# liangyuwang/Tiny-DeepSpeed

Hardware: AMD Instinct MI355X
Metric: tokens/sec (whole node) GPT-2 ZeRO-2 (higher is better)
Workload: dtype bf16; 1 GPU; model=gpt2-medium, global_batch=32, seq_len=1024, parallelism=zero2-dp1

## Files before the change

### csrc/kernels/attention.hip

```cpp
#include "common.h"
#include "launchers.h"
#include "mfma.h"

#include <type_traits>

namespace tdsa {

constexpr int KVB = 64;
constexpr int D = 64;
constexpr float LOG2E = 1.4426950408889634f;
constexpr float LN2 = 0.6931471805599453f;

DEV_INLINE float fast_exp2(float x) { return __builtin_amdgcn_exp2f(x); }
DEV_INLINE float fast_rcp(float x) { return __builtin_amdgcn_rcpf(x); }

DEV_INLINE void xcd_remap(int gx, long long gy, int& tile, long long& bh) {
  if (gy % 8 == 0) {
    const long long id = bh * gx + tile;
    tile = (int)((id % (8 * gx)) / 8);
    bh = (id / (8 * gx)) * 8 + (id % 8);
  }
}

struct GStride {
  long long b;
  long long h;
  int t;
};

struct BlockCtx {
  int tile;
  long long bh;
  int tid, lane, w;
  int x32, h32;

  DEV_INLINE BlockCtx() {
    tile = blockIdx.x;
    bh = blockIdx.y;
    xcd_remap(gridDim.x, gridDim.y, tile, bh);
    tid = threadIdx.x;
    lane = tid & (WAVE - 1);
    w = tid / WAVE;
    x32 = lane & 31;
    h32 = lane >> 5;
  }

  DEV_INLINE long long base(const GStride& s, int H) const {
    return (bh / H) * s.b + (bh % H) * s.h;
  }
};

struct FragOff {
  int row[2];
  int xk;
  int h16;

  DEV_INLINE FragOff(const BlockCtx& c)
      : row{c.x32 * 128, (32 + c.x32) * 128}, xk((c.x32 & 7) << 4),
        h16(16 * c.h32) {}

  DEV_INLINE int operator()(int t2, int s) const {
    return row[t2] + ((s * 32 + h16) ^ xk);
  }
};

template <int NT>
struct TilePipe {
  Stage<NT> a, b;
  short8v pend_a[Stage<NT>::REPS], pend_b[Stage<NT>::REPS];

  DEV_INLINE TilePipe(const bf16* ga, int st_a, const bf16* gb, int st_b,
                      int tid)
      : a(ga, tid, st_a), b(gb, tid, st_b) {}

  DEV_INLINE void prime() {
    a.fetch(pend_a);
    b.fetch(pend_b);
  }

  DEV_INLINE void next(char* lds_a, char* lds_b, bool more) {
    __syncthreads();
    a.put(lds_a, pend_a);
    b.put(lds_b, pend_b);
    if (more) {
      a.advance();
      b.advance();
      a.fetch(pend_a);
      b.fetch(pend_b);
    }
  }
};

struct Dropout {
  unsigned long long seed;
  unsigned keep_thr;
  float inv_keep;

  DEV_INLINE bool keep(unsigned long long idx) const {
    unsigned h = (unsigned)(idx ^ (idx >> 32));
    h += (unsigned)seed;
    h ^= (unsigned)(seed >> 32);
    h ^= h >> 16;
    h *= 0x85EBCA6Bu;
    h ^= h >> 13;
    h *= 0xC2B2AE35u;
    h ^= h >> 16;
    return h < keep_thr;
  }
};

struct PackedC {
  unsigned wA[2][4];
  unsigned wB[2][4];
};

DEV_INLINE bfrag frag_from_packed(const PackedC& p, int s) {
  const unsigned uA = p.wA[s >> 1][2 * (s & 1)];
  const unsigned vA = p.wA[s >> 1][2 * (s & 1) + 1];
  const unsigned uB = p.wB[s >> 1][2 * (s & 1)];
  const unsigned vB = p.wB[s >> 1][2 * (s & 1) + 1];
  auto rA = __builtin_amdgcn_permlane32_swap(uA, vA, false, false);
  auto rB = __builtin_amdgcn_permlane32_swap(uB, vB, false, false);
  union { bfrag f; unsigned w[4]; } r;
  r.w[0] = rA[0];
  r.w[1] = rB[0];
  r.w[2] = rA[1];
  r.w[3] = rB[1];
  return r.f;
}

DEV_INLINE bfrag load_frag_scaled(const bf16* p, int row, int col, int st,
                                  float s) {
  short8v v = load8(p + (long long)row * st + col);
  union { bfrag f; short w[8]; } r;
#pragma unroll
  for (int e = 0; e < 8; ++e) r.w[e] = bf_pack(bf_elem(v, e) * s);
  return r.f;
}

DEV_INLINE bfrag load_frag(const bf16* p, int row, int col, int st) {
  union { bfrag f; short8v v; } r;
  r.v = load8(p + (long long)row * st + col);
  return r.f;
}

template <typename F>
DEV_INLINE void store_ctiles(bf16* p, int st, const BlockCtx& c,
                             const f32x16 (&acc)[2], F mul) {
#pragma unroll
  for (int dt = 0; dt < 2; ++dt)
#pragma unroll
    for (int r = 0; r < 16; ++r)
      p[crow(r, c.h32) * st + dt * 32 + c.x32] = f2bf(acc[dt][r] * mul(r));
}

constexpr int fwd_min_blocks(int nw, bool drop) {
  return nw == 8 ? (drop ? 3 : 4) : 2;
}

template <int NW, bool DROP = false>
__launch_bounds__(NW * WAVE, fwd_min_blocks(NW, DROP))
__global__ void attn_fwd_kernel(const bf16* __restrict__ q,
                                const bf16* __restrict__ k,
                                const bf16* __restrict__ v,
                                bf16* __restrict__ o, float* __restrict__ lse,
                                int T, int H, float scale, GStride sq,
                                GStride so, Dropout drop) {
  constexpr int BM = NW * 32;
  constexpr int NT = NW * WAVE;
  __shared__ __attribute__((aligned(16))) char smem[2 * KVB * D * 2];
  char* lds_k = smem;
  char* lds_v = smem + KVB * D * 2;

  const BlockCtx c;
  const long long boff = c.base(sq, H);
  const bf16* qp = q + boff + (long long)(c.tile * BM) * sq.t;

  TilePipe<NT> pipe(k + boff, sq.t, v + boff, sq.t, c.tid);
  const FragOff kf(c);
  int trb[2][2];
  tr_bases(c.lane, trb);
  const float qscale = scale * LOG2E;
  bfrag q_frag[4];
#pragma unroll
  for (int s = 0; s < 4; ++s)
    q_frag[s] = load_frag_scaled(qp, c.w * 32 + c.x32, s * 16 + 8 * c.h32,
                                 sq.t, qscale);

  const f32x16 kzero = {};
  f32x16 o_acc[2] = {};
  float m_run = -INFINITY;
  float l_run = 0.f;

  const int row_lo = c.tile * BM + c.w * 32;
  const int row_me = row_lo + c.x32;
  const unsigned long long drop_base =
      DROP ? ((unsigned long long)c.bh * T + row_me) * T : 0;
  const int n_kv = (c.tile + 1) * BM / KVB;
  pipe.prime();
  for (int j = 0; j < n_kv; ++j) {
    pipe.next(lds_k, lds_v, j + 1 < n_kv);
    __syncthreads();

    const int key0 = j * KVB;
    if (key0 > row_lo + 31) continue;

    f32x16 st[2];
    __builtin_amdgcn_s_setprio(1);
#pragma unroll
    for (int t2 = 0; t2 < 2; ++t2) {
      f32x16 acc = MFMA32(lds_read16(lds_k, kf(t2, 0)), q_frag[0], kzero);
#pragma unroll
      for (int s = 1; s < 4; ++s)
        acc = MFMA32(lds_read16(lds_k, kf(t2, s)), q_frag[s], acc);
      st[t2] = acc;
    }
    __builtin_amdgcn_s_setprio(0);

    const bool diag = key0 + KVB - 1 > row_lo;
    float mt = -INFINITY;
    if (diag) {
#pragma unroll
      for (int t2 = 0; t2 < 2; ++t2)
#pragma unroll
        for (int r = 0; r < 16; ++r) {
          const int key = key0 + t2 * 32 + crow(r, c.h32);
          float s = (key <= row_me) ? st[t2][r] : -INFINITY;
          st[t2][r] = s;
          mt = fmaxf(mt, s);
        }
    } else {
#pragma unroll
      for (int t2 = 0; t2 < 2; ++t2)
#pragma unroll
        for (int r = 0; r < 16; ++r) mt = fmaxf(mt, st[t2][r]);
    }
    mt = fmaxf(mt, __shfl_xor(mt, 32, WAVE));
    const float m_new = fmaxf(m_run, mt);
    const float alpha = fast_exp2(m_run - m_new);
    float psum = 0.f;
    PackedC P;
#pragma unroll
    for (int t2 = 0; t2 < 2; ++t2)
#pragma unroll
      for (int r1 = 0; r1 < 4; ++r1) {
        float p[4];
#pragma unroll
        for (int e = 0; e < 4; ++e) {
          float pe = fast_exp2(st[t2][4 * r1 + e] - m_new);
          psum += pe;
          if (DROP) {
            const int key = key0 + t2 * 32 + crow(4 * r1 + e, c.h32);
            pe = drop.keep(drop_base + key) ? pe * drop.inv_keep : 0.f;
          }
          p[e] = pe;
        }
        P.wA[t2][r1] = pack2(p[0], p[1]);
        P.wB[t2][r1] = pack2(p[2], p[3]);
      }
    psum += __shfl_xor(psum, 32, WAVE);
    l_run = l_run * alpha + psum;
    m_run = m_new;

    if (__any(alpha != 1.0f)) {
      float a_row[16];
#pragma unroll
      for (int r = 0; r < 16; ++r)
        a_row[r] = __shfl(alpha, crow(r, c.h32), WAVE);
#pragma unroll
      for (int dt = 0; dt < 2; ++dt)
#pragma unroll
        for (int r = 0; r < 16; ++r) o_acc[dt][r] *= a_row[r];
    }

    __builtin_amdgcn_s_setprio(1);
#pragma unroll
    for (int s = 0; s < 4; ++s) {
      const bfrag pa = frag_from_packed(P, s);
#pragma unroll
      for (int dt = 0; dt < 2; ++dt)
        o_acc[dt] = MFMA32(pa, tr_bfrag(lds_v, trb[dt][0] + s * 2048,
                                        trb[dt][1] + s * 2048),
                           o_acc[dt]);
    }
    __builtin_amdgcn_s_setprio(0);
  }

  float linv_row[16];
#pragma unroll
  for (int r = 0; r < 16; ++r)
    linv_row[r] = fast_rcp(__shfl(l_run, crow(r, c.h32), WAVE));
  store_ctiles(o + c.base(so, H) + (long long)row_lo * so.t, so.t, c, o_acc,
               [&](int r) { return linv_row[r]; });
  if (c.lane < 32) {
    lse[c.bh * T + row_me] = (m_run + log2f(l_run)) * LN2;
  }
}

template <int NW, bool DROP = false>
__launch_bounds__(NW * WAVE)
__global__ void attn_bwd_dkv_kernel(const bf16* __restrict__ q,
                                    const bf16* __restrict__ k,
                                    const bf16* __restrict__ v,
                                    const bf16* __restrict__ dout,
                                    const float* __restrict__ lse,
                                    const float* __restrict__ delta,
                                    bf16* __restrict__ dk, bf16* __restrict__ dv,
                                    int T, int H, float scale, GStride sq,
                                    GStride so, GStride sd, Dropout drop) {
  constexpr int BK = NW * 32;
  constexpr int NT = NW * WAVE;
  __shared__ __attribute__((aligned(16))) char smem[2 * KVB * D * 2 + 2 * KVB * 4];
  char* lds_q = smem;
  char* lds_do = smem + KVB * D * 2;
  float* lds_lse = reinterpret_cast<float*>(smem + 2 * KVB * D * 2);
  float* lds_dlt = lds_lse + KVB;

  const BlockCtx c;
  const long long boff = c.base(sq, H);
  const int i0 = c.tile * BK / KVB;

  TilePipe<NT> pipe(q + boff + (long long)(i0 * KVB) * sq.t, sq.t,
                    dout + c.base(so, H) + (long long)(i0 * KVB) * so.t, so.t,
                    c.tid);
  const FragOff af(c);
  int trb[2][2];
  tr_bases(c.lane, trb);
  const float kscale = scale * LOG2E;
  const int key_lo = c.tile * BK + c.w * 32;
  const int key_me = key_lo + c.x32;
  const unsigned long long drop_bhTT =
      DROP ? (unsigned long long)c.bh * T * T : 0;
  bfrag k_frag[4], v_frag[4];
#pragma unroll
  for (int s = 0; s < 4; ++s) {
    k_frag[s] = load_frag_scaled(k + boff, key_me, s * 16 + 8 * c.h32, sq.t,
                                 kscale);
    v_frag[s] = load_frag(v + boff, key_me, s * 16 + 8 * c.h32, sq.t);
  }

  const f32x16 kzero = {};
  f32x16 dk_acc[2] = {};
  f32x16 dv_acc[2] = {};

  pipe.prime();
  for (int i = i0; i < T / KVB; ++i) {
    pipe.next(lds_q, lds_do, i + 1 < T / KVB);
    if (c.tid < KVB) {
      lds_lse[c.tid] = lse[c.bh * T + i * KVB + c.tid] * LOG2E;
      lds_dlt[c.tid] = delta[c.bh * T + i * KVB + c.tid];
    }
    __syncthreads();

    const int q0 = i * KVB;
    if (q0 + KVB - 1 < key_lo) continue;

    const bool diag = q0 < key_lo + 32;
    PackedC P, dS;
#pragma unroll
    for (int t2 = 0; t2 < 2; ++t2) {
      __builtin_amdgcn_s_setprio(1);
      f32x16 s_acc = MFMA32(lds_read16(lds_q, af(t2, 0)), k_frag[0], kzero);
      f32x16 dp_acc = MFMA32(lds_read16(lds_do, af(t2, 0)), v_frag[0], kzero);
#pragma unroll
      for (int s = 1; s < 4; ++s) {
        s_acc = MFMA32(lds_read16(lds_q, af(t2, s)), k_frag[s], s_acc);
        dp_acc = MFMA32(lds_read16(lds_do, af(t2, s)), v_frag[s], dp_acc);
      }
      __builtin_amdgcn_s_setprio(0);
      auto consume = [&](auto MASK) {
#pragma unroll
        for (int r1 = 0; r1 < 4; ++r1) {
          float p[4], dsv[4];
#pragma unroll
          for (int e = 0; e < 4; ++e) {
            const int r = 4 * r1 + e;
            const int lrow = t2 * 32 + crow(r, c.h32);
            float pp = fast_exp2(s_acc[r] - lds_lse[lrow]);
            if (MASK.value) pp = (key_me <= q0 + lrow) ? pp : 0.f;
            float pv = pp;
            float dpv = dp_acc[r];
            if (DROP) {
              const bool keep = drop.keep(
                  drop_bhTT + (unsigned)((q0 + lrow) * T) + key_me);
              pv = keep ? pp * drop.inv_keep : 0.f;
              dpv = keep ? dpv * drop.inv_keep : 0.f;
            }
            p[e] = pv;
            dsv[e] = pp * (dpv - lds_dlt[lrow]);
          }
          P.wA[t2][r1] = pack2(p[0], p[1]);
          P.wB[t2][r1] = pack2(p[2], p[3]);
          dS.wA[t2][r1] = pack2(dsv[0], dsv[1]);
          dS.wB[t2][r1] = pack2(dsv[2], dsv[3]);
        }
      };
      if (diag)
        consume(std::true_type{});
      else
        consume(std::false_type{});
    }

    __builtin_amdgcn_s_setprio(1);
#pragma unroll
    for (int s = 0; s < 4; ++s) {
      const bfrag ap = frag_from_packed(P, s);
      const bfrag as = frag_from_packed(dS, s);
#pragma unroll
      for (int dt = 0; dt < 2; ++dt) {
        dv_acc[dt] = MFMA32(ap, tr_bfrag(lds_do, trb[dt][0] + s * 2048,
                                         trb[dt][1] + s * 2048),
                            dv_acc[dt]);
        dk_acc[dt] = MFMA32(as, tr_bfrag(lds_q, trb[dt][0] + s * 2048,
                                         trb[dt][1] + s * 2048),
                            dk_acc[dt]);
      }
    }
    __builtin_amdgcn_s_setprio(0);
  }

  const long long doff = c.base(sd, H) + (long long)(key_lo) * sd.t;
  bf16* dkp = dk + doff;
  bf16* dvp = dv + doff;
#pragma unroll
  for (int dt = 0; dt < 2; ++dt)
#pragma unroll
    for (int r = 0; r < 16; ++r) {
      dkp[crow(r, c.h32) * sd.t + dt * 32 + c.x32] = f2bf(dk_acc[dt][r] * scale);
      dvp[crow(r, c.h32) * sd.t + dt * 32 + c.x32] = f2bf(dv_acc[dt][r]);
    }
}

template <int NW, bool DROP = false>
__launch_bounds__(NW * WAVE)
__global__ void attn_bwd_dq_kernel(const bf16* __restrict__ q,
                                   const bf16* __restrict__ k,
                                   const bf16* __restrict__ v,
                                   const bf16* __restrict__ o,
                                   const bf16* __restrict__ dout,
                                   const float* __restrict__ lse,
                                   float* __restrict__ delta,
                                   bf16* __restrict__ dq, int T, int H,
                                   float scale, GStride sq, GStride so,
                                   GStride sd, Dropout drop) {
  constexpr int BM = NW * 32;
  constexpr int NT = NW * WAVE;
  __shared__ __attribute__((aligned(16))) char smem[2 * KVB * D * 2];
  char* lds_k = smem;
  char* lds_v = smem + KVB * D * 2;

  const BlockCtx c;
  const long long boff = c.base(sq, H);
  const long long ooff = c.base(so, H) + (long long)(c.tile * BM) * so.t;
  const bf16* qp = q + boff + (long long)(c.tile * BM) * sq.t;

  TilePipe<NT> pipe(k + boff, sq.t, v + boff, sq.t, c.tid);
  const FragOff fo(c);
  int f_off[2][4];
#pragma unroll
  for (int t2 = 0; t2 < 2; ++t2)
#pragma unroll
    for (int s = 0; s < 4; ++s) f_off[t2][s] = fo(t2, s);
  int trb[2][2];
  tr_bases(c.lane, trb);
  const float qscale = scale * LOG2E;
  bfrag q_frag[4], do_frag[4];
#pragma unroll
  for (int s = 0; s < 4; ++s) {
    q_frag[s] = load_frag_scaled(qp, c.w * 32 + c.x32, s * 16 + 8 * c.h32,
                                 sq.t, qscale);
    do_frag[s] = load_frag(dout + ooff, c.w * 32 + c.x32, s * 16 + 8 * c.h32,
                           so.t);
  }
  const int row_lo = c.tile * BM + c.w * 32;
  const int row_me = row_lo + c.x32;
  const unsigned long long drop_base =
      DROP ? ((unsigned long long)c.bh * T + row_me) * T : 0;
  const float lse2_me = lse[c.bh * T + row_me] * LOG2E;
  float dlt_me = 0.f;
#pragma unroll
  for (int s = 0; s < 4; ++s) {
    union { bfrag f; short8v v8; } ov;
    ov.f = load_frag(o + ooff, c.w * 32 + c.x32, s * 16 + 8 * c.h32, so.t);
    union { bfrag f; short8v v8; } dv;
    dv.f = do_frag[s];
#pragma unroll
    for (int e = 0; e < 8; ++e)
      dlt_me += bf_elem(ov.v8, e) * bf_elem(dv.v8, e);
  }
  dlt_me += __shfl_xor(dlt_me, 32, WAVE);
  if (c.lane < 32) delta[c.bh * T + row_me] = dlt_me;

  const f32x16 kzero = {};
  f32x16 dq_acc[2] = {};

  const int n_kv = (c.tile + 1) * BM / KVB;
  pipe.prime();
  for (int j = 0; j < n_kv; ++j) {
    pipe.next(lds_k, lds_v, j + 1 < n_kv);
    __syncthreads();

    const int key0 = j * KVB;
    if (key0 > row_lo + 31) continue;

    const bool diag = key0 + KVB - 1 > row_lo;
    PackedC dS;
#pragma unroll
    for (int t2 = 0; t2 < 2; ++t2) {
      __builtin_amdgcn_s_setprio(1);
      f32x16 s_acc = MFMA32(lds_read16(lds_k, f_off[t2][0]), q_frag[0], kzero);
      f32x16 dp_acc = MFMA32(lds_read16(lds_v, f_off[t2][0]), do_frag[0], kzero);
#pragma unroll
      for (int s = 1; s < 4; ++s) {
        s_acc = MFMA32(lds_read16(lds_k, f_off[t2][s]), q_frag[s], s_acc);
        dp_acc = MFMA32(lds_read16(lds_v, f_off[t2][s]), do_frag[s], dp_acc);
      }
      __builtin_amdgcn_s_setprio(0);
      float dsv[16];
      auto consume = [&](auto MASK) {
#pragma unroll
        for (int r = 0; r < 16; ++r) {
          float pp = fast_exp2(s_acc[r] - lse2_me);
          if (MASK.value) {
            const int key = key0 + t2 * 32 + crow(r, c.h32);
            pp = (key <= row_me) ? pp : 0.f;
          }
          float dpv = dp_acc[r];
          if (DROP) {
            const int key = key0 + t2 * 32 + crow(r, c.h32);
            dpv = drop.keep(drop_base + key) ? dpv * drop.inv_keep : 0.f;
          }
          dsv[r] = pp * (dpv - dlt_me);
        }
      };
      if (diag)
        consume(std::true_type{});
      else
        consume(std::false_type{});
#pragma unroll
      for (int r1 = 0; r1 < 4; ++r1) {
        dS.wA[t2][r1] = pack2(dsv[4 * r1], dsv[4 * r1 + 1]);
        dS.wB[t2][r1] = pack2(dsv[4 * r1 + 2], dsv[4 * r1 + 3]);
      }
    }

    __builtin_amdgcn_s_setprio(1);
#pragma unroll
    for (int s = 0; s < 4; ++s) {
      const bfrag as = frag_from_packed(dS, s);
#pragma unroll
      for (int dt = 0; dt < 2; ++dt)
        dq_acc[dt] = MFMA32(as, tr_bfrag(lds_k, trb[dt][0] + s * 2048,
                                         trb[dt][1] + s * 2048),
                            dq_acc[dt]);
    }
    __builtin_amdgcn_s_setprio(0);
  }

  store_ctiles(dq + c.base(sd, H) + (long long)row_lo * sd.t, sd.t, c, dq_acc,
               [&](int) { return scale; });
}

static GStride gstride(const long long* s) { return {s[0], s[1], (int)s[2]}; }

static Dropout make_dropout(float p, unsigned long long seed) {
  const double keepd = 1.0 - (double)p;
  const double thr_d = keepd * 4294967296.0;
  const unsigned keep_thr =
      thr_d >= 4294967295.0 ? 0xFFFFFFFFu : (unsigned)thr_d;
  return {seed, keep_thr, (float)(1.0 / keepd)};
}

template <typename F>
static void attn_dispatch(int T, const char* nw_env, bool drop, F f) {
  const long long knob = env_int(nw_env, 8);
  const int nw_max = (knob == 2 || knob == 4) ? (int)knob : 8;
  auto with_nw = [&](auto DROP) {
    if (T % 256 == 0 && nw_max == 8) f(std::integral_constant<int, 8>{}, DROP);
    else if (T % 128 == 0 && nw_max >= 4) f(std::integral_constant<int, 4>{}, DROP);
    else f(std::integral_constant<int, 2>{}, DROP);
  };
  if (drop) with_nw(std::true_type{}); else with_nw(std::false_type{});
}

}

using namespace tdsa;

extern "C" {

hipError_t tdsa_attn_fwd(const void* q, const void* k, const void* v, void* o,
                         float* lse, long long B, long long H, int T,
                         float scale, const long long* sq_in,
                         const long long* so_in, float dropout_p,
                         unsigned long long seed, hipStream_t stream) {
  if (T % KVB) return hipErrorInvalidValue;
  const GStride sq = gstride(sq_in), so = gstride(so_in);
  const Dropout drop = make_dropout(dropout_p, seed);
  attn_dispatch(T, "TDSA_ATTN_FWD_NW", dropout_p > 0.0f, [&](auto nw, auto dr) {
    constexpr int NW = decltype(nw)::value;
    hipLaunchKernelGGL((attn_fwd_kernel<NW, decltype(dr)::value>),
                       dim3(T / (NW * 32), B * H), dim3(NW * WAVE), 0, stream,
                       (const bf16*)q, (const bf16*)k, (const bf16*)v,
                       (bf16*)o, lse, T, (int)H, scale, sq, so, drop);
  });
  return hipGetLastError();
}

hipError_t tdsa_attn_bwd(const void* q, const void* k, const void* v,
                         const void* o, const float* lse, const void* dout,
                         void* dq, void* dk, void* dv, float* delta,
                         long long B, long long H, int T, float scale,
                         const long long* sq_in, const long long* so_in,
                         const long long* sd_in, float dropout_p,
                         unsigned long long seed, hipStream_t stream) {
  if (T % KVB) return hipErrorInvalidValue;
  const GStride sq = gstride(sq_in), so = gstride(so_in), sd = gstride(sd_in);
  const Dropout drop = make_dropout(dropout_p, seed);
  attn_dispatch(T, "TDSA_ATTN_BWD_NW", dropout_p > 0.0f, [&](auto nw, auto dr) {
    constexpr int NW = decltype(nw)::value;
    constexpr bool DROP = decltype(dr)::value;
    const dim3 grid(T / (NW * 32), B * H), block(NW * WAVE);
    hipLaunchKernelGGL((attn_bwd_dq_kernel<NW, DROP>), grid, block, 0, stream,
                       (const bf16*)q, (const bf16*)k, (const bf16*)v,
                       (const bf16*)o, (const bf16*)dout, lse, delta,
                       (bf16*)dq, T, (int)H, scale, sq, so, sd, drop);
    hipLaunchKernelGGL((attn_bwd_dkv_kernel<NW, DROP>), grid, block, 0, stream,
                       (const bf16*)q, (const bf16*)k, (const bf16*)v,
                       (const bf16*)dout, lse, delta, (bf16*)dk, (bf16*)dv, T,
                       (int)H, scale, sq, so, sd, drop);
  });
  return hipGetLastError();
}

}
```

### csrc/kernels/mfma.h

```cpp
#pragma once

#include "common.h"

#define MFMA32(a, b, c) \
  __builtin_amdgcn_mfma_f32_32x32x16_bf16((a), (b), (c), 0, 0, 0)

namespace tdsa {

typedef __attribute__((ext_vector_type(8))) short bfrag;
typedef __attribute__((__vector_size__(4 * sizeof(__bf16)))) __bf16 bf16x4v;
#define LDS_AS __attribute__((address_space(3)))

DEV_INLINE int swz(int row, int byte_in_row) {
  return row * 128 + (byte_in_row ^ ((row & 7) << 4));
}

DEV_INLINE unsigned pack2(float lo, float hi) {
  union { struct { short a, b; } s; unsigned u; } u;
  u.s.a = bf_pack(lo);
  u.s.b = bf_pack(hi);
  return u.u;
}

DEV_INLINE bfrag lds_read16(const char* lds, int byte_off) {
  return *reinterpret_cast<const bfrag*>(lds + byte_off);
}

DEV_INLINE int crow(int r, int h32) { return (r & 3) + 8 * (r >> 2) + 4 * h32; }

template <int NT>
struct Stage {
  static constexpr int REPS = 512 / NT;
  const bf16* src[REPS];
  int dst[REPS];
  long long step;

  DEV_INLINE Stage() {}

  DEV_INLINE Stage(const bf16* g, int tid, long long t_stride, int rows = 64) {
    init(g, tid, t_stride, rows);
  }

  DEV_INLINE void init(const bf16* g, int tid, long long t_stride,
                       int rows = 64) {
    step = (long long)rows * t_stride;
#pragma unroll
    for (int rep = 0; rep < REPS; ++rep) {
      int chunk = tid + rep * NT;
      src[rep] = g + (long long)(chunk >> 3) * t_stride + (chunk & 7) * 8;
      dst[rep] = swz(chunk >> 3, (chunk & 7) * 16);
    }
  }

  DEV_INLINE void run(char* lds) {
#pragma unroll
    for (int rep = 0; rep < REPS; ++rep)
      *reinterpret_cast<short8v*>(lds + dst[rep]) = load8(src[rep]);
  }

  DEV_INLINE void advance() {
#pragma unroll
    for (int rep = 0; rep < REPS; ++rep) src[rep] += step;
  }

  DEV_INLINE void fetch(short8v (&buf)[REPS]) {
#pragma unroll
    for (int rep = 0; rep < REPS; ++rep) buf[rep] = load8(src[rep]);
  }

  DEV_INLINE void put(char* lds, const short8v (&buf)[REPS]) {
#pragma unroll
    for (int rep = 0; rep < REPS; ++rep)
      *reinterpret_cast<short8v*>(lds + dst[rep]) = buf[rep];
  }
};

DEV_INLINE bfrag tr_bfrag(const char* lds, int a_lo, int a_hi) {
  bf16x4v lo = __builtin_amdgcn_ds_read_tr16_b64_v4bf16(
      (LDS_AS bf16x4v*)(lds + a_lo));
  bf16x4v hi = __builtin_amdgcn_ds_read_tr16_b64_v4bf16(
      (LDS_AS bf16x4v*)(lds + a_hi));
  union { bfrag f; bf16x4v h[2]; } r;
  r.h[0] = lo;
  r.h[1] = hi;
  return r.f;
}

DEV_INLINE void tr_bases(int lane, int (&trb)[2][2]) {
  const int g4 = lane >> 4;
  const int i = lane & 15;
  const int hh = g4 >> 1;
  const int iq = i >> 2;
#pragma unroll
  for (int dt = 0; dt < 2; ++dt)
#pragma unroll
    for (int half = 0; half < 2; ++half) {
      const int row = 8 * hh + 4 * half + iq;
      const int colbyte = (dt * 32 + 16 * (g4 & 1) + 4 * (i & 3)) * 2;
      trb[dt][half] = row * 128 + (colbyte ^ ((row & 7) << 4));
    }
}

}
```

Baseline: 337,900 tokens/s.

## Software-pipeline LDS operand reads against MFMAs in attention backward kernels

Adds an OperandRing that prefetches LDS fragments a fixed depth ahead of each MFMA, with sched_group_barrier hints that interleave reads with matrix ops in both the dK/dV and dQ backward kernels. The dK/dV and dQ accumulation MFMAs move inside the per-half t2 loop, so each half's output products overlap the next half's score computation. The lse/delta row loads are also prefetched one iteration ahead through a register pipeline and read as 4-wide vectors. The aim is to hide LDS and global latency behind MFMA work, at the cost of more live registers, which could lower occupancy or cause spills.

```diff
diff --git a/csrc/kernels/attention.hip b/csrc/kernels/attention.hip
--- a/csrc/kernels/attention.hip
+++ b/csrc/kernels/attention.hip
@@ -8,6 +8,7 @@
 
 constexpr int KVB = 64;
 constexpr int D = 64;
+constexpr int RING = 4;
 constexpr float LOG2E = 1.4426950408889634f;
 constexpr float LN2 = 0.6931471805599453f;
 
@@ -87,6 +88,38 @@
       b.advance();
       a.fetch(pend_a);
       b.fetch(pend_b);
+    }
+  }
+};
+
+struct RowPipe {
+  const float* x;
+  const float* y;
+  float pend_x, pend_y;
+  int row;
+  bool loader;
+
+  DEV_INLINE RowPipe(const float* gx, const float* gy, int tid)
+      : x(gx + tid), y(gy + tid), pend_x(0.f), pend_y(0.f), row(tid),
+        loader(tid < KVB) {}
+
+  DEV_INLINE void prime() {
+    if (loader) {
+      pend_x = *x;
+      pend_y = *y;
+    }
+  }
+
+  DEV_INLINE void next(float* lds_x, float* lds_y, float mul_x, bool more) {
+    if (loader) {
+      lds_x[row] = pend_x * mul_x;
+      lds_y[row] = pend_y;
+      if (more) {
+        x += KVB;
+        y += KVB;
+        pend_x = *x;
+        pend_y = *y;
+      }
     }
   }
 };
@@ -323,6 +356,7 @@
   TilePipe<NT> pipe(q + boff + (long long)(i0 * KVB) * sq.t, sq.t,
                     dout + c.base(so, H) + (long long)(i0 * KVB) * so.t, so.t,
                     c.tid);
+  RowPipe rows(lse + c.bh * T + i0 * KVB, delta + c.bh * T + i0 * KVB, c.tid);
   const FragOff af(c);
   int trb[2][2];
   tr_bases(c.lane, trb);
@@ -344,12 +378,11 @@
   f32x16 dv_acc[2] = {};
 
   pipe.prime();
+  rows.prime();
   for (int i = i0; i < T / KVB; ++i) {
-    pipe.next(lds_q, lds_do, i + 1 < T / KVB);
-    if (c.tid < KVB) {
-      lds_lse[c.tid] = lse[c.bh * T + i * KVB + c.tid] * LOG2E;
-      lds_dlt[c.tid] = delta[c.bh * T + i * KVB + c.tid];
-    }
+    const bool more = i + 1 < T / KVB;
+    pipe.next(lds_q, lds_do, more);
+    rows.next(lds_lse, lds_dlt, LOG2E, more);
     __syncthreads();
 
     const int q0 = i * KVB;
@@ -357,26 +390,48 @@
 
     const bool diag = q0 < key_lo + 32;
     PackedC P, dS;
+    auto sdp_operand = [&](int t2) {
+      return [&, t2](int n) {
+        return lds_read16((n & 1) ? lds_do : lds_q, af(t2, n >> 1));
+      };
+    };
+    OperandRing<RING> sdp_ring;
+    sdp_ring.prime(sdp_operand(0));
 #pragma unroll
     for (int t2 = 0; t2 < 2; ++t2) {
+      const int row4 = 32 * t2 + 4 * c.h32;
+      f32x4 lse4 = Vec<float, 4>::load(lds_lse + row4);
+      f32x4 dlt4 = Vec<float, 4>::load(lds_dlt + row4);
       __builtin_amdgcn_s_setprio(1);
-      f32x16 s_acc = MFMA32(lds_read16(lds_q, af(t2, 0)), k_frag[0], kzero);
-      f32x16 dp_acc = MFMA32(lds_read16(lds_do, af(t2, 0)), v_frag[0], kzero);
-#pragma unroll
-      for (int s = 1; s < 4; ++s) {
-        s_acc = MFMA32(lds_read16(lds_q, af(t2, s)), k_frag[s], s_acc);
-        dp_acc = MFMA32(lds_read16(lds_do, af(t2, s)), v_frag[s], dp_acc);
-      }
+      f32x16 s_acc = kzero, dp_acc = kzero;
+      sdp_ring.template run<8, 1>(sdp_operand(t2), [&](int n, bfrag a) {
+        if (n & 1)
+          dp_acc = MFMA32(a, v_frag[n >> 1], dp_acc);
+        else
+          s_acc = MFMA32(a, k_frag[n >> 1], s_acc);
+      });
       __builtin_amdgcn_s_setprio(0);
+      auto out_operand = [&](int n) {
+        const int off = (2 * t2 + (n >> 2)) * 2048, dt = (n >> 1) & 1;
+        return tr_bfrag((n & 1) ? lds_q : lds_do, trb[dt][0] + off,
+                        trb[dt][1] + off);
+      };
+      OperandRing<RING> out_ring;
+      out_ring.prime(out_operand);
       auto consume = [&](auto MASK) {
 #pragma unroll
         for (int r1 = 0; r1 < 4; ++r1) {
+          const f32x4 lse_g = lse4, dlt_g = dlt4;
+          if (r1 < 3) {
+            lse4 = Vec<float, 4>::load(lds_lse + row4 + 8 * (r1 + 1));
+            dlt4 = Vec<float, 4>::load(lds_dlt + row4 + 8 * (r1 + 1));
+          }
           float p[4], dsv[4];
 #pragma unroll
           for (int e = 0; e < 4; ++e) {
             const int r = 4 * r1 + e;
             const int lrow = t2 * 32 + crow(r, c.h32);
-            float pp = fast_exp2(s_acc[r] - lds_lse[lrow]);
+            float pp = fast_exp2(s_acc[r] - lse_g[e]);
             if (MASK.value) pp = (key_me <= q0 + lrow) ? pp : 0.f;
             float pv = pp;
             float dpv = dp_acc[r];
@@ -387,7 +442,7 @@
               dpv = keep ? dpv * drop.inv_keep : 0.f;
             }
             p[e] = pv;
-            dsv[e] = pp * (dpv - lds_dlt[lrow]);
+            dsv[e] = pp * (dpv - dlt_g[e]);
           }
           P.wA[t2][r1] = pack2(p[0], p[1]);
           P.wB[t2][r1] = pack2(p[2], p[3]);
@@ -399,24 +454,23 @@
         consume(std::true_type{});
       else
         consume(std::false_type{});
-    }
-
-    __builtin_amdgcn_s_setprio(1);
-#pragma unroll
-    for (int s = 0; s < 4; ++s) {
-      const bfrag ap = frag_from_packed(P, s);
-      const bfrag as = frag_from_packed(dS, s);
-#pragma unroll
-      for (int dt = 0; dt < 2; ++dt) {
-        dv_acc[dt] = MFMA32(ap, tr_bfrag(lds_do, trb[dt][0] + s * 2048,
-                                         trb[dt][1] + s * 2048),
-                            dv_acc[dt]);
-        dk_acc[dt] = MFMA32(as, tr_bfrag(lds_q, trb[dt][0] + s * 2048,
-                                         trb[dt][1] + s * 2048),
-                            dk_acc[dt]);
-      }
-    }
-    __builtin_amdgcn_s_setprio(0);
+
+      if (t2 == 0) sdp_ring.prime(sdp_operand(1));
+
+      __builtin_amdgcn_s_setprio(1);
+      const bfrag ap[2] = {frag_from_packed(P, 2 * t2),
+                           frag_from_packed(P, 2 * t2 + 1)};
+      const bfrag as[2] = {frag_from_packed(dS, 2 * t2),
+                           frag_from_packed(dS, 2 * t2 + 1)};
+      out_ring.template run<8, 2>(out_operand, [&](int n, bfrag b) {
+        const int dt = (n >> 1) & 1;
+        if (n & 1)
+          dk_acc[dt] = MFMA32(as[n >> 2], b, dk_acc[dt]);
+        else
+          dv_acc[dt] = MFMA32(ap[n >> 2], b, dv_acc[dt]);
+      });
+      __builtin_amdgcn_s_setprio(0);
+    }
   }
 
   const long long doff = c.base(sd, H) + (long long)(key_lo) * sd.t;
@@ -505,17 +559,30 @@
 
     const bool diag = key0 + KVB - 1 > row_lo;
     PackedC dS;
+    auto sdp_operand = [&](int t2) {
+      return [&, t2](int n) {
+        return lds_read16((n & 1) ? lds_v : lds_k, f_off[t2][n >> 1]);
+      };
+    };
+    OperandRing<RING> sdp_ring;
+    sdp_ring.prime(sdp_operand(0));
 #pragma unroll
     for (int t2 = 0; t2 < 2; ++t2) {
       __builtin_amdgcn_s_setprio(1);
-      f32x16 s_acc = MFMA32(lds_read16(lds_k, f_off[t2][0]), q_frag[0], kzero);
-      f32x16 dp_acc = MFMA32(lds_read16(lds_v, f_off[t2][0]), do_frag[0], kzero);
-#pragma unroll
-      for (int s = 1; s < 4; ++s) {
-        s_acc = MFMA32(lds_read16(lds_k, f_off[t2][s]), q_frag[s], s_acc);
-        dp_acc = MFMA32(lds_read16(lds_v, f_off[t2][s]), do_frag[s], dp_acc);
-      }
+      f32x16 s_acc = kzero, dp_acc = kzero;
+      sdp_ring.template run<8, 1>(sdp_operand(t2), [&](int n, bfrag a) {
+        if (n & 1)
+          dp_acc = MFMA32(a, do_frag[n >> 1], dp_acc);
+        else
+          s_acc = MFMA32(a, q_frag[n >> 1], s_acc);
+      });
       __builtin_amdgcn_s_setprio(0);
+      auto out_operand = [&](int n) {
+        const int off = (2 * t2 + (n >> 1)) * 2048, dt = n & 1;
+        return tr_bfrag(lds_k, trb[dt][0] + off, trb[dt][1] + off);
+      };
+      OperandRing<RING> out_ring;
+      out_ring.prime(out_operand);
       float dsv[16];
       auto consume = [&](auto MASK) {
 #pragma unroll
@@ -542,19 +609,17 @@
         dS.wA[t2][r1] = pack2(dsv[4 * r1], dsv[4 * r1 + 1]);
         dS.wB[t2][r1] = pack2(dsv[4 * r1 + 2], dsv[4 * r1 + 3]);
       }
-    }
-
-    __builtin_amdgcn_s_setprio(1);
-#pragma unroll
-    for (int s = 0; s < 4; ++s) {
-      const bfrag as = frag_from_packed(dS, s);
-#pragma unroll
-      for (int dt = 0; dt < 2; ++dt)
-        dq_acc[dt] = MFMA32(as, tr_bfrag(lds_k, trb[dt][0] + s * 2048,
-                                         trb[dt][1] + s * 2048),
-                            dq_acc[dt]);
-    }
-    __builtin_amdgcn_s_setprio(0);
+
+      if (t2 == 0) sdp_ring.prime(sdp_operand(1));
+
+      __builtin_amdgcn_s_setprio(1);
+      const bfrag as[2] = {frag_from_packed(dS, 2 * t2),
+                           frag_from_packed(dS, 2 * t2 + 1)};
+      out_ring.template run<4, 2>(out_operand, [&](int n, bfrag b) {
+        dq_acc[n & 1] = MFMA32(as[n >> 1], b, dq_acc[n & 1]);
+      });
+      __builtin_amdgcn_s_setprio(0);
+    }
   }
 
   store_ctiles(dq + c.base(sd, H) + (long long)row_lo * sd.t, sd.t, c, dq_acc,
diff --git a/csrc/kernels/mfma.h b/csrc/kernels/mfma.h
--- a/csrc/kernels/mfma.h
+++ b/csrc/kernels/mfma.h
@@ -86,6 +86,31 @@
   return r.f;
 }
 
+template <int DEPTH>
+struct OperandRing {
+  bfrag slot[DEPTH];
+
+  template <typename R>
+  DEV_INLINE void prime(R read) {
+#pragma unroll
+    for (int n = 0; n < DEPTH; ++n) slot[n] = read(n);
+  }
+
+  template <int N, int READS, typename R, typename M>
+  DEV_INLINE void run(R read, M mma) {
+#pragma unroll
+    for (int n = 0; n < N; ++n) {
+      const bfrag op = slot[n % DEPTH];
+      if (n + DEPTH < N) {
+        slot[n % DEPTH] = read(n + DEPTH);
+        __builtin_amdgcn_sched_group_barrier(0x100, READS, 0);
+      }
+      mma(n, op);
+      __builtin_amdgcn_sched_group_barrier(0x008, 1, 0);
+    }
+  }
+};
+
 DEV_INLINE void tr_bases(int lane, int (&trb)[2][2]) {
   const int g4 = lane >> 4;
   const int i = lane & 15;
```

After: 341,000 tokens/s (median of 3 runs). About the same (+0.9%).

## Prefetch LSE/delta rows in attention backward pipeline and use packed bf16 conversion

Applied to the files above, without the earlier changes.

Adds a RowPipe that prefetches the per-tile LSE and delta rows into registers alongside the Q/dO tile pipeline, so the global loads overlap with compute instead of being issued after the barrier. It also hoists the causal-mask and dropout row-index arithmetic out of the inner loop, and pins some values in VGPRs to stop the compiler from rematerialising them. pack2 now uses a vector float-to-bf16 convertvector, which may lower to a hardware packed conversion instead of two scalar bf_pack calls. This costs extra registers in the backward kernel, and the rounding behaviour may differ from the old bf_pack.

```diff
diff --git a/csrc/kernels/attention.hip b/csrc/kernels/attention.hip
--- a/csrc/kernels/attention.hip
+++ b/csrc/kernels/attention.hip
@@ -13,6 +13,8 @@
 
 DEV_INLINE float fast_exp2(float x) { return __builtin_amdgcn_exp2f(x); }
 DEV_INLINE float fast_rcp(float x) { return __builtin_amdgcn_rcpf(x); }
+DEV_INLINE float pin(float x) { asm("" : "+v"(x)); return x; }
+DEV_INLINE unsigned pin(unsigned x) { asm("" : "+v"(x)); return x; }
 
 DEV_INLINE void xcd_remap(int gx, long long gy, int& tile, long long& bh) {
   if (gy % 8 == 0) {
@@ -79,15 +81,62 @@
   }
 
   DEV_INLINE void next(char* lds_a, char* lds_b, bool more) {
+    next(lds_a, lds_b, more, NoRows{});
+  }
+
+  template <typename Rows>
+  DEV_INLINE void next(char* lds_a, char* lds_b, bool more, Rows&& rows) {
     __syncthreads();
     a.put(lds_a, pend_a);
     b.put(lds_b, pend_b);
+    rows.put();
     if (more) {
       a.advance();
       b.advance();
       a.fetch(pend_a);
       b.fetch(pend_b);
-    }
+      rows.advance();
+      rows.fetch();
+    }
+  }
+
+  struct NoRows {
+    DEV_INLINE void put() {}
+    DEV_INLINE void advance() {}
+    DEV_INLINE void fetch() {}
+  };
+};
+
+struct RowPipe {
+  const float* ga;
+  const float* gb;
+  float* lds_a;
+  float* lds_b;
+  float mul_a;
+  int tid;
+  float pend_a, pend_b;
+
+  DEV_INLINE RowPipe(const float* ga, const float* gb, float* lds_a,
+                     float* lds_b, float mul_a, int tid)
+      : ga(ga), gb(gb), lds_a(lds_a), lds_b(lds_b), mul_a(mul_a), tid(tid) {}
+
+  DEV_INLINE void fetch() {
+    if (tid < KVB) {
+      pend_a = ga[tid];
+      pend_b = gb[tid];
+    }
+  }
+
+  DEV_INLINE void put() {
+    if (tid < KVB) {
+      lds_a[tid] = pend_a * mul_a;
+      lds_b[tid] = pend_b;
+    }
+  }
+
+  DEV_INLINE void advance() {
+    ga += KVB;
+    gb += KVB;
   }
 };
 
@@ -251,7 +300,7 @@
           psum += pe;
           if (DROP) {
             const int key = key0 + t2 * 32 + crow(4 * r1 + e, c.h32);
-            pe = drop.keep(drop_base + key) ? pe * drop.inv_keep : 0.f;
+            pe = pin(drop.keep(drop_base + key) ? pe * drop.inv_keep : 0.f);
           }
           p[e] = pe;
         }
@@ -343,19 +392,21 @@
   f32x16 dk_acc[2] = {};
   f32x16 dv_acc[2] = {};
 
+  const long long row0 = c.bh * T + i0 * KVB;
+  RowPipe rows(lse + row0, delta + row0, lds_lse, lds_dlt, LOG2E, c.tid);
   pipe.prime();
+  rows.fetch();
   for (int i = i0; i < T / KVB; ++i) {
-    pipe.next(lds_q, lds_do, i + 1 < T / KVB);
-    if (c.tid < KVB) {
-      lds_lse[c.tid] = lse[c.bh * T + i * KVB + c.tid] * LOG2E;
-      lds_dlt[c.tid] = delta[c.bh * T + i * KVB + c.tid];
-    }
+    pipe.next(lds_q, lds_do, i + 1 < T / KVB, rows);
     __syncthreads();
 
     const int q0 = i * KVB;
     if (q0 + KVB - 1 < key_lo) continue;
 
     const bool diag = q0 < key_lo + 32;
+    const int mask_lo = key_me - q0 - 4 * c.h32;
+    const unsigned drop_rowT =
+        DROP ? pin((unsigned)((q0 + 4 * c.h32) * T)) : 0;
     PackedC P, dS;
 #pragma unroll
     for (int t2 = 0; t2 < 2; ++t2) {
@@ -377,12 +428,14 @@
             const int r = 4 * r1 + e;
             const int lrow = t2 * 32 + crow(r, c.h32);
             float pp = fast_exp2(s_acc[r] - lds_lse[lrow]);
-            if (MASK.value) pp = (key_me <= q0 + lrow) ? pp : 0.f;
+            if (MASK.value) pp = (t2 * 32 + crow(r, 0) >= mask_lo) ? pp : 0.f;
             float pv = pp;
             float dpv = dp_acc[r];
             if (DROP) {
               const bool keep = drop.keep(
-                  drop_bhTT + (unsigned)((q0 + lrow) * T) + key_me);
+                  drop_bhTT +
+                  (drop_rowT + (unsigned)((t2 * 32 + crow(r, 0)) * T)) +
+                  key_me);
               pv = keep ? pp * drop.inv_keep : 0.f;
               dpv = keep ? dpv * drop.inv_keep : 0.f;
             }
diff --git a/csrc/kernels/mfma.h b/csrc/kernels/mfma.h
--- a/csrc/kernels/mfma.h
+++ b/csrc/kernels/mfma.h
@@ -15,10 +15,13 @@
   return row * 128 + (byte_in_row ^ ((row & 7) << 4));
 }
 
+typedef __attribute__((ext_vector_type(2))) float f32x2;
+typedef __attribute__((ext_vector_type(2))) __bf16 bf16x2v;
+
 DEV_INLINE unsigned pack2(float lo, float hi) {
-  union { struct { short a, b; } s; unsigned u; } u;
-  u.s.a = bf_pack(lo);
-  u.s.b = bf_pack(hi);
+  const f32x2 f = {lo, hi};
+  union { bf16x2v h; unsigned u; } u;
+  u.h = __builtin_convertvector(f, bf16x2v);
   return u.u;
 }
 
```

New measurement: 324,300 tokens/s before, 334,500 tokens/s after, median of 6. 1.03x the previous value.
